# 1005088h/3d_object_detection

Measured on AMD Instinct MI355X. Metric: point-cloud frames/sec end-to-end (voxelise→NMS), eight_20cm, 1x MI355X, higher is better.
Workload: dtype f32; 1 GPU; configs/eight_20cm.json, synthetic KITTI-shape 64-beam 20k-point clouds (mean 20000 points, one distinct cloud per frame of a step), independent frames (batch=1 semantics), random-init weights (InstanceNorm backbone), AABB NMS; `value`: clouds resident in HBM; frames_per_pass_per_gpu=32, engine_max_batch=32, parallelism=frame-sharded x1

## Files before the change

3d_object_detection_amd/csrc/conv.hip:

```cpp
#include <algorithm>
#include <type_traits>
#include <cmath>
#include <cstdio>
#include <cstdlib>
#include <cstring>
#include <unistd.h>
#include "pp_common.h"
#include "conv_common.h"

namespace {

using namespace ppc;

__global__ void __launch_bounds__(256) norm_relu_stats(const float* __restrict__ x, float* __restrict__ y, int C, int HW,
                                                       int pre, const double* __restrict__ pre_acc,
                                                       const float* __restrict__ pre_scale, const float* __restrict__ pre_shift,
                                                       double inv_n, float eps, double* __restrict__ stat_acc,
                                                       size_t x_fs, size_t acc_fs, int x16, int y16)
{
    const int c = blockIdx.y;
    const _Float16* xh = reinterpret_cast<const _Float16*>(x) + blockIdx.z * x_fs;
    _Float16* yh = reinterpret_cast<_Float16*>(y) + blockIdx.z * x_fs;
    x += blockIdx.z * x_fs;
    y += blockIdx.z * x_fs;
// ... 441 lines not shown
        p.feat_fs = (size_t)ctx->cfg.max_voxels * 64;
    }
    const bool fin_in_kernel = B == 1 && finalises_in_prologue(L.var.family);
    if (pre.mode == PRE_STATS && net->aff && L.cin <= 320 && !fin_in_kernel) {
        hipLaunchKernelGGL(norm_finalize, dim3(B), dim3(320), 0, stream, pre.acc, pre.fs, L.cin, pre.inv_n, p.eps, net->aff, (size_t)640);
        p.pre = PRE_AFFINE; p.pre_scale = net->aff; p.pre_shift = net->aff + 320; p.aff_fs = 640;
    }
    const Variant& v = L.var;
    const bool tag = ctx->prof_on && L.kind == 0 && L.level == 0 && L.stride == 1;
    auto prof_begin = [&]() -> int {
        if (!tag) return 0;
        if (ctx->prof_used + 2 > ctx->prof_ev.size()) {
            hipEvent_t a, b;
            PP_HIP(hipEventCreate(&a));
            PP_HIP(hipEventCreate(&b));
            ctx->prof_ev.push_back(a);
            ctx->prof_ev.push_back(b);
        }
        ctx->prof_flops = 2.0 * Hout * Wout * (double)L.cin * L.cout * 9.0 * B;
        PP_HIP(hipEventRecord(ctx->prof_ev[ctx->prof_used], stream));
        return 0;
    };
    auto prof_end = [&]() -> int {
        if (!tag) return 0;
        PP_HIP(hipEventRecord(ctx->prof_ev[ctx->prof_used + 1], stream));
        ctx->prof_used += 2;
        return 0;
    };
    dim3 grid(pp_div_up(Wout, v.pw) * pp_div_up(Hout, v.ph), pp_div_up(L.rows, v.bm), B);
    p.nb = B;
    const size_t lds_bytes = layer_lds(v, L.cin);
    if (v.family == Family::Gemm1x1 && ((Hin * Win) & 3)) return PP_E_ARG;
    if (v.family == Family::Gemm1x1) {
        const int ncb = pp_div_up(L.rows, v.bm);
        int g = (net->num_cu * v.wpc / ncb) * ncb;
        if (g < ncb) g = ncb;
        grid = dim3(g, 1, 1);
    }
    if (v.family == Family::Conv16) {
        if ((size_t)L.rows * Hout * Wout * 4 >= 0x80000000ull || (size_t)L.cin * Hin * Win * 4 >= 0x80000000ull) return PP_E_ARG;
        if (p.pre == PRE_STATS) return pp_fail(ctx, PP_E_STATE, "conv16: the producer's statistics must be finalised to (scale, shift)");
        if ((Win & 3) || (Wout & 3) || (L.cin & 15) || (L.rows % v.bm)) return PP_E_ARG;
        const int total = pp_div_up(Wout, v.pw) * pp_div_up(Hout, v.ph) * (L.rows / v.bm) * B;
        int g = net->num_cu * (v.waves * 64 / v.threads);

        if (g > total) g = total;
        g = (g + 7) & ~7;
        grid = dim3(g, 1, 1);
    }
    if (v.family == Family::Wino4 || v.family == Family::Wino6) {
        if ((size_t)L.rows * Hout * Wout * 4 >= 0x80000000ull) return PP_E_ARG;
        if (p.pre == PRE_RAW) return pp_fail(ctx, PP_E_ARG, "wino4 / wino6 tilings have no raw prologue: give the layer a (scale, shift)");
        const int ncb = pp_div_up(L.rows, v.bm);
        const int2* ts_items = nullptr;
        const int32_t* ts_count = nullptr;
        const bool listed = ts_k > 0 && v.family == Family::Wino6 && v.kern2 && v.pw == 16 && v.ph == 16 && net->eff_prec == 0 && !net->up16 &&
                            L.kind == 0 && L.level == 0 && L.stride == 1 && Wout % v.pw == 0 && Hout % v.ph == 0 && Hout == ctx->H && Wout == ctx->W &&
                            pp_ts_list(ctx, ts_k, B, &ts_items, &ts_count);
        if (tag) {
            const double dense = (double)(Wout / v.pw) * (Hout / v.ph) * ncb * B;
            ctx->prof_items_dense += dense;
            if (listed) ctx->prof_ts_layer.push_back(ts_k | (ncb << 8)); else ctx->prof_items += dense;
        }
        if (int rc = prof_begin()) return rc;
        auto launch_region = [&](const Variant& rv, int x0, int y0, int x1, int y1) {
            ConvP q = p;
// ... 8 lines not shown
        };
        const int mw = (Wout / v.pw) * v.pw, mh = (Hout / v.ph) * v.ph;
        const Variant &sv = strip_v(v.family), &sh = strip_h(v.family);
        const int plan_b = ctx->max_batch;
        auto rounds = [&](int tiles) { return tiles > 0 ? pp_div_up((int64_t)tiles * ncb * plan_b, net->num_cu) : 0; };
        const int t_main = (mw / v.pw) * (mh / v.ph);
        const int t_right = Wout > mw ? pp_div_up(Wout - mw, sv.pw) * pp_div_up(Hout, sv.ph) : 0;
        const int t_bottom = Hout > mh ? pp_div_up(mw, sh.pw) * pp_div_up(Hout - mh, sh.ph) : 0;
        const double tile_us = v.family == Family::Wino6 ? 1.9 * (L.cin / 8) + 3.5 : 2.4 * (L.cin / 8) + 5.0;
        const double full = rounds(pp_div_up(Wout, v.pw) * pp_div_up(Hout, v.ph)) * tile_us;
        const double split = (rounds(t_main) + rounds(t_right) + rounds(t_bottom)) * tile_us + 30.0 * ((t_right > 0) + (t_bottom > 0));
        const bool no_strips = net->w4_strips == 0, all_strips = net->w4_strips == 2;
        if ((split < full || all_strips) && mw > 0 && mh > 0 && !no_strips && (Wout > mw || Hout > mh)) {
            launch_region(v, 0, 0, mw, mh);
            if (Wout > mw) launch_region(sv, mw, 0, Wout, Hout);
            if (Hout > mh) launch_region(sh, 0, mh, mw, Hout);
        } else {
            launch_region(v, 0, 0, Wout, Hout);
            if (listed)
                if (int rc = pp_ts_fill(ctx, ts_k, B, out, p.out_fs, L.rows, stream)) return rc;
        }
        if (int rc = prof_end()) return rc;
        PP_HIP(hipGetLastError());
        return 0;
    }
    if (v.family == Family::Wino) {
        const int total = (int)grid.x * (int)grid.y * B;
        int g = (v.threads >= 512 ? 1 : 2) * net->num_cu;
        if (g > total) g = total;
        g = (g + 7) & ~7;
        grid = dim3(g, 1, 1);
    }
    if (int rc = prof_begin()) return rc;
    hipLaunchKernelGGL((pmap && v.kern2) ? v.kern2 : v.kern, grid, dim3(v.threads), lds_bytes, stream, p);
    if (int rc = prof_end()) return rc;
    PP_HIP(hipGetLastError());
    return 0;
}


__global__ void __launch_bounds__(256) f32_to_f16(const float* __restrict__ x, _Float16* __restrict__ y, size_t n)
{
    for (size_t i = (size_t)blockIdx.x * blockDim.x + threadIdx.x; i < n; i += (size_t)gridDim.x * blockDim.x) y[i] = (_Float16)x[i];
}

__global__ void __launch_bounds__(256) fill_pattern(float* __restrict__ x, size_t n)
{
    for (size_t i = (size_t)blockIdx.x * blockDim.x + threadIdx.x; i < n; i += (size_t)gridDim.x * blockDim.x) {
        unsigned h = (unsigned)i * 2654435761u;
        h ^= h >> 15; h *= 2246822519u; h ^= h >> 13;
        x[i] = (float)(h & 0xFFFF) * (1.0f / 65536.0f);
    }
}

std::map<std::string, std::string>& tune_cache()
{
    static std::map<std::string, std::string> c;
    static bool loaded = false;
    if (!loaded) {
        loaded = true;
        if (const char* path = getenv("PP_TUNE_CACHE")) {
            if (FILE* f = fopen(path, "r")) {
                char line[512];
                while (fgets(line, sizeof(line), f)) {
                    char* tab = strchr(line, '\t');
                    if (!tab) continue;
                    *tab = 0;
// ... 228 lines not shown
    PP_HIP(hipMalloc((void**)&net->bn_scale, (size_t)24 * 320 * sizeof(float)));
    PP_HIP(hipMalloc((void**)&net->bn_shift, (size_t)24 * 320 * sizeof(float)));
    PP_HIP(hipMalloc((void**)&net->head_bias, (size_t)head_rows(ctx->cfg.num_anchor_per_loc) * sizeof(float)));
    PP_HIP(hipMalloc((void**)&net->head_bias_perm, 96 * sizeof(float)));
    PP_HIP(hipMalloc((void**)&net->ones, 320 * sizeof(float)));
    PP_HIP(hipMalloc((void**)&net->zeros, 320 * sizeof(float)));
    std::vector<float> one(320, 1.f);
    PP_HIP(hipMemcpy(net->ones, one.data(), 320 * sizeof(float), hipMemcpyHostToDevice));
    PP_HIP(hipMemset(net->zeros, 0, 320 * sizeof(float)));
    int cin = 64;
    for (int b = 0; b < 3; ++b) {
        const int c = kC[b];
        const int nres[3] = {1, 1, 0};
        const int nunits = (b == 0) ? 2 : 3;
        char key[128];
        snprintf(key, sizeof(key), "rpn.block%d.0.weight", b + 1);
        net->layers.push_back(Layer{key, 0, cin, c, 2, 1, b, pick_variant(0, 2, 1, c, H >> b, W >> b)});
        for (int u = 0; u < nunits; ++u) {
            const int nl = (b == 0) ? (u == 0 ? 1 : 0) : nres[u];
            snprintf(key, sizeof(key), "rpn.block%d.%d.conv_block.2.weight", b + 1, 3 + u);
            net->layers.push_back(Layer{key, 0, c, c, 1, 1, b, pick_variant(0, 1, 1, c, H >> b, W >> b)});
            if (nl == 1) {
                snprintf(key, sizeof(key), "rpn.block%d.%d.conv_block.5.weight", b + 1, 3 + u);
                net->layers.push_back(Layer{key, 0, c, c, 1, 1, b, pick_variant(0, 1, 1, c, H >> b, W >> b)});
            }
        }
        const int up = 1 << b;
        snprintf(key, sizeof(key), "rpn.deconv%d.0.weight", b + 1);
        net->layers.push_back(Layer{key, 1, c, (b == 0) ? 64 : 128, 1, up, b, pick_variant(1, 1, up, ((b == 0) ? 64 : 128) * up * up, H >> b, W >> b)});
        cin = c;
    }
    net->layers.push_back(Layer{"heads", 2, 320, 10 * ctx->cfg.num_anchor_per_loc, 1, 1, 0,
                                pick_variant(2, 1, 1, head_rows(ctx->cfg.num_anchor_per_loc), H, W, ctx->cfg.num_anchor_per_loc == 9)});
    for (Layer& L : net->layers)
        PP_HIP(hipFuncSetAttribute((const void*)L.var.kern, hipFuncAttributeMaxDynamicSharedMemorySize, (int)L.var.lds));
    for (Family f : {Family::Wino4, Family::Wino6})
        for (const Variant* sv : {&strip_v(f), &strip_h(f)})
            PP_HIP(hipFuncSetAttribute((const void*)sv->kern, hipFuncAttributeMaxDynamicSharedMemorySize, (int)sv->lds));
    return 0;
}

void pp_net_destroy(pp_ctx* ctx)
{
    pp_net* net = (pp_net*)ctx->net;
    if (!net) return;
    for (int l = 0; l < 3; ++l)
        for (int b = 0; b < 4; ++b)
            if (net->buf[l][b]) (void)hipFree(net->buf[l][b] - W6_FRONT_PAD);
    for (Layer& L : net->layers)
        if (L.w) (void)hipFree(L.w);
    void* ptrs[] = {net->dbg_stats, net->up, net->stats, net->aff, net->bn_scale, net->bn_shift, net->head_bias, net->head_bias_perm, net->ones, net->zeros};
    for (void* q : ptrs)
        if (q) (void)hipFree(q);
    delete net;
    ctx->net = nullptr;
}

static int fold_bn(pp_ctx* ctx, const std::string& prefix, int C, int site)
{
    pp_net* net = (pp_net*)ctx->net;
    auto get = [&](const char* s) -> const std::vector<float>* {
        auto it = ctx->host_w.find(prefix + s);
        if (it == ctx->host_w.end() || (int)it->second.data.size() != C) return nullptr;
        return &it->second.data;
    };
    const std::vector<float>*g = get(".weight"), *b = get(".bias"), *rm = get(".running_mean"), *rv = get(".running_var");
    if (!g || !b || !rm || !rv) return pp_fail(ctx, PP_E_NAME, ("missing BatchNorm tensors for " + prefix).c_str());
    std::vector<float> sc(C), sh(C);
// ... 30 lines not shown
        float hp[96];
        for (int t = 0; t < 96; ++t) hp[t] = head_tile_row(t) >= 0 ? hb[head_tile_row(t)] : 0.f;
        PP_HIP(hipMemcpy(net->head_bias_perm, hp, sizeof(hp), hipMemcpyHostToDevice));
    }
    {
        const char* at = getenv("PP_AUTOTUNE");
        const char* vb = getenv("PP_VERBOSE");
        const bool tune = !(at && at[0] == '0');
        const bool verbose = vb && vb[0] != '0';
        const int H = ctx->H, W = ctx->W;
        float *tin = nullptr, *tout = nullptr;
        const bool can_tune = tune && (H % 4 == 0) && (W % 4 == 0);
        net->up16 = ctx->precision == 4 && (W % 16 == 0) && ((H * W) % 64 == 0) && ctx->cfg.num_anchor_per_loc == 9;
        net->eff_prec = (ctx->precision == 4 && !net->up16) ? 3 : ctx->precision;
        if (can_tune) {
            const size_t nin = std::max((size_t)64 * ctx->gx * ctx->gy, (size_t)320 * H * W);
            const int tb = ctx->max_batch < TUNE_FRAMES ? ctx->max_batch : TUNE_FRAMES;
            PP_HIP(hipMalloc((void**)&tin, ((size_t)tb * nin + 256 + W6_FRONT_PAD) * sizeof(float)));
            tin += W6_FRONT_PAD;
            PP_HIP(hipMalloc((void**)&tout, ((size_t)tb * 320 * H * W + 256) * sizeof(float)));
            hipLaunchKernelGGL(fill_pattern, dim3(2048), dim3(256), 0, 0, tin, (size_t)tb * nin);
        }
        for (Layer& L : net->layers) {
            int rc = 0;
            {
                const int h = H >> L.level, w = W >> L.level;
                const int hin = (L.kind == 0 && L.stride == 2) ? h * 2 : h, win = (L.kind == 0 && L.stride == 2) ? w * 2 : w;
                if (!can_tune && net->eff_prec == 0) L.var = pick_variant(L.kind, L.stride, L.up, (L.kind == 2) ? head_rows(ctx->cfg.num_anchor_per_loc) : (L.kind == 1 ? L.cout * L.up * L.up : L.cout), h, w, ctx->cfg.num_anchor_per_loc == 9);
                rc = autotune_layer(ctx, L, hin, win, h, w, tin, tout, verbose, can_tune);
                if (rc) { if (tin) { (void)hipFree(tin - W6_FRONT_PAD); (void)hipFree(tout); } return rc; }
            }
            PP_HIP(hipFuncSetAttribute((const void*)L.var.kern, hipFuncAttributeMaxDynamicSharedMemorySize,
                                       (int)layer_lds(L.var, L.cin)));
            if (L.var.kern2) PP_HIP(hipFuncSetAttribute((const void*)L.var.kern2, hipFuncAttributeMaxDynamicSharedMemorySize, (int)L.var.lds));
            rc = pack_layer(ctx, L);
            if (rc) { if (tin) { (void)hipFree(tin - W6_FRONT_PAD); (void)hipFree(tout); } return rc; }
        }
        ctx->sc1_kc = (net->layers[0].var.family == Family::Direct && net->layers[0].var.kc == 8) ? 8 : 4;
        {
            const Layer& head = net->layers.back();
            net->defer_ok = net->eff_prec == 0 && na == 9 && head.var.family == Family::Gemm1x1 && head.var.prec == 0 && head.var.io16 == 0;
            if (net->defer_ok) {
                const int rc = autotune_head_cls(ctx, tin, verbose, can_tune);
                if (rc) { if (tin) { (void)hipFree(tin - W6_FRONT_PAD); (void)hipFree(tout); } return rc; }
            }
        }
        if (tin) { PP_HIP(hipDeviceSynchronize()); (void)hipFree(tin - W6_FRONT_PAD); (void)hipFree(tout); tune_cache_save(); }
        if (net->up16)
            for (const Layer& L : net->layers)
                if ((L.kind == 1 && L.var.io16 != 3) || (L.kind == 2 && L.var.io16 != 1) ||
                    (L.kind == 0 && L.var.io16 != ((L.stride == 2 && L.level == 0) ? 2 : 3)))
                    return pp_fail(ctx, PP_E_STATE, "fp16s: a layer did not get a 16-bit-tensor tiling (PP_FORCE_VARIANT?)");
    }
    if (ctx->cfg.norm_kind == 1) {
        for (int b = 0; b < 3; ++b) {
            char key[128];
            const int c = kC[b];
            snprintf(key, sizeof(key), "rpn.block%d.1", b + 1);
            int rc = fold_bn(ctx, key, c, site_block(b, 0));
            if (rc) return rc;
            const int nunits = (b == 0) ? 2 : 3;
            for (int u = 0; u < nunits; ++u) {
                const int nl = (u == nunits - 1) ? 0 : 1;
                snprintf(key, sizeof(key), "rpn.block%d.%d.conv_block.0", b + 1, 3 + u);
                if ((rc = fold_bn(ctx, key, c, site_block(b, 1 + 2 * u)))) return rc;
                if (nl) {
                    snprintf(key, sizeof(key), "rpn.block%d.%d.conv_block.3", b + 1, 3 + u);
// ... 675 lines not shown
```

3d_object_detection_amd/csrc/gemm1x1.hip:

```cpp
#include <cstdio>
#include "pp_common.h"
#include "conv_common.h"

namespace {

using namespace ppc;

typedef short s16x4 __attribute__((ext_vector_type(4)));
typedef __bf16 bf16x2_t __attribute__((ext_vector_type(2)));
__device__ __forceinline__ unsigned pk_bf16(float a, float b)
{
    return __builtin_bit_cast(unsigned, __builtin_convertvector((f32x2_t){a, b}, bf16x2_t));
}
template <int PREC>
__device__ __forceinline__ f32x4 mfma_lp(const s16x4 a, const s16x4 b, const f32x4 c)
{
    if constexpr (PREC == 3) return __builtin_amdgcn_mfma_f32_16x16x16f16(__builtin_bit_cast(f16x4_t, a), __builtin_bit_cast(f16x4_t, b), c, 0, 0, 0);
    else return __builtin_amdgcn_mfma_f32_16x16x16bf16_1k(a, b, c, 0, 0, 0);
}

template <int MT, int NT, int EPI, int PREC = 0, int IO16 = 0, int PDX = 0>
__global__ void __launch_bounds__(512, EPI == EPI_HEAD_CLS ? 4 : 2) gemm1x1(const ConvP p)
{
    constexpr bool IN16 = (IO16 & 1) != 0, OUT16 = (IO16 & 2) != 0;
    static_assert(IO16 == 0 || PREC != 0, "16-bit storage comes with the 16-bit operand path");
    static_assert(!OUT16 || EPI != EPI_HEAD, "the head's logits stay fp32");
    constexpr int BM = MT * 16;
    constexpr int BMP = BM + ((BM % 32 == 0) ? 16 : 0);
    static_assert(EPI != EPI_HEAD_CLS || (MT == 1 && PREC == 0 && IO16 == 0), "the cls-only head pass is one fp32 M-tile");
    constexpr int PD = PDX ? PDX : (MT >= 8) ? 4 : 8;
    extern __shared__ __attribute__((aligned(16))) float smem[];
    float* wl = smem;
    const int K = p.Cin;
    float* sc_all = wl + (size_t)K * BMP;
    const int tid = threadIdx.x, lane = tid & 63, wave = __builtin_amdgcn_readfirstlane(tid >> 6);
    const int m = lane & 15, kq = lane >> 4;
    float* scl = sc_all + (size_t)wave * 2 * K;
    float* shl = scl + K;

    const int ncb = (p.Cout + BM - 1) / BM;
    const bool xcd_ok = gridDim.x % (8 * ncb) == 0;
    const int xj = blockIdx.x >> 3, xk = blockIdx.x & 7;
    const int cb = xcd_ok ? xj % ncb : blockIdx.x % ncb;
    const int wi = xcd_ok ? xk + 8 * (xj / ncb) : blockIdx.x / ncb, nworkers = gridDim.x / ncb;
    if (wi >= nworkers) return;
    const int co0 = cb * BM;
    if constexpr (EPI == EPI_HEAD_CLS) {
        for (int e = tid; e < K * BMP; e += 512) {
            const int k = e / BMP, a = e - k * BMP, t = 4 * (9 + a) + 3;
            wl[e] = a < p.n_cls ? p.w[((size_t)(t / p.w_bm) * K + k) * p.w_bmp + t % p.w_bm] : 0.f;
        }
    } else {
        const f32x4* g = reinterpret_cast<const f32x4*>(p.w) + (size_t)cb * ((size_t)K * BMP / 4);
        f32x4* d = reinterpret_cast<f32x4*>(wl);
        for (int e = tid; e < K * BMP / 4; e += 512) d[e] = g[e];
    }
// ... 23 lines not shown
                float s = ssum[i][r], q = ssq[i][r];
                s = row16_sum(s);
                q = row16_sum(q);
                const int row = co0 + i * 16 + kq * 4 + r;
                int ch = row;
                bool lead = (m == 0);
                if (EPI == EPI_UP2) { ch = row >> 2; lead = lead && r == 0; }
                if (EPI == EPI_UP4) { ch = row >> 4; lead = lead && r == 0; }
                if (lead && row < p.Cout) {
                    atomicAdd(base + (size_t)ch * 2, (double)s);
                    atomicAdd(base + (size_t)ch * 2 + 1, (double)q);
                }
                ssum[i][r] = 0.f;
                ssq[i][r] = 0.f;
            }
    };

    const int aoff = kq * BMP + m;
    static_assert(NT == 4, "gemm1x1 is written for 4 interleaved N-tiles");
    const int nsteps = K / 4;
    const unsigned bstep = 16u * (unsigned)plane;
    __amdgpu_buffer_rsrc_t rb = __builtin_amdgcn_make_buffer_rsrc(const_cast<float*>(p.in), 0, 0x7FFFFFFF, 0x00020000);
    unsigned bvoff = 0u;
    f32x4 bq[PD];
    auto set_load_item = [&](int it) {
        const int f_ = __builtin_amdgcn_readfirstlane(it / items_per_frame);
        const int px_ = __builtin_amdgcn_readfirstlane((it - f_ * items_per_frame) * (NT * 16)) + 4 * m;
        const uint64_t bp_ = IN16 ? (uint64_t)(reinterpret_cast<const _Float16*>(p.in) + (size_t)f_ * p.in_fs) : (uint64_t)(p.in + (size_t)f_ * p.in_fs);
        const uint64_t bps_ = ((uint64_t)(uint32_t)__builtin_amdgcn_readfirstlane((int)(bp_ >> 32)) << 32) | (uint32_t)__builtin_amdgcn_readfirstlane((int)(uint32_t)bp_);
        rb = __builtin_amdgcn_make_buffer_rsrc(reinterpret_cast<float*>(bps_), 0, 0x7FFFFFFF, 0x00020000);
        bvoff = ((unsigned)kq * (unsigned)plane + (unsigned)(px_ < HW ? px_ : 0)) * (IN16 ? 2u : 4u);
    };
#define G1_LOADB(S, SLOT) bq[SLOT] = __builtin_bit_cast(f32x4, __builtin_amdgcn_raw_buffer_load_b128(rb, bvoff, (unsigned)(S) * bstep, 0));
#define G1_PREP(S, SLOT, PAR)                                                                    \
    {                                                                                            \
        _Pragma("unroll") for (int i = 0; i < MT; ++i) a[PAR][i] = wl[(S) * 4 * BMP + aoff + i * 16]; \
        if (p.pre != PRE_RAW) {                                                                  \
            const float sc = scl[(S) * 4 + kq], sh = shl[(S) * 4 + kq];                          \
            _Pragma("unroll") for (int j = 0; j < NT; ++j) b[PAR][j] = fmaxf(fmaf(bq[SLOT][j], sc, sh), 0.f); \
        } else {                                                                                 \
            _Pragma("unroll") for (int j = 0; j < NT; ++j) b[PAR][j] = bq[SLOT][j];              \
        }                                                                                        \
    }
#define G1_MFMAS(PAR)                                                                            \
    {                                                                                            \
        __builtin_amdgcn_sched_barrier(0);                                                       \
        _Pragma("unroll") for (int i = 0; i < MT; ++i)                                           \
            _Pragma("unroll") for (int j = 0; j < NT; ++j)                                       \
                acc[i][j] = __builtin_amdgcn_mfma_f32_16x16x4f32(a[PAR][i], b[PAR][j], acc[i][j], 0, 0, 0); \
        __builtin_amdgcn_sched_barrier(0);                                                       \
    }
    if constexpr (PREC == 0) {
    if (gw < total) {
        set_load_item(gw);
#pragma unroll
        for (int s0 = 0; s0 < PD - 1; ++s0) G1_LOADB(s0, s0)
    }
    }
    for (int item = gw; item < total; item += gstride) {
        const int fr = __builtin_amdgcn_readfirstlane(item / items_per_frame);
        const int pix0 = __builtin_amdgcn_readfirstlane((item - fr * items_per_frame) * (NT * 16));
        if (fr != stat_frame) { flush_stats(stat_frame); stat_frame = fr; }
        if (p.pre != PRE_RAW && fr != pre_frame) {
            for (int c = lane; c < K; c += 64) {
                if (p.pre == PRE_STATS) {
                    const double* pa = p.pre_acc + (size_t)fr * p.pre_fs;
                    double s = 0.0, q = 0.0;
#pragma unroll
                    for (int r = 0; r < NREP; ++r) { s += pa[((size_t)r * K + c) * 2]; q += pa[((size_t)r * K + c) * 2 + 1]; }
                    const double mean = s * p.pre_inv_n;
                    double var = q * p.pre_inv_n - mean * mean;
                    var = var > 0.0 ? var : 0.0;
                    const double rstd = 1.0 / sqrt(var + (double)p.eps);
                    scl[c] = (float)rstd;
                    shl[c] = (float)(-mean * rstd);
                } else {
                    scl[c] = p.pre_scale[(size_t)fr * p.aff_fs + c];
                    shl[c] = p.pre_shift[(size_t)fr * p.aff_fs + c];
                }
            }
            pre_frame = fr;
        }
        const int pxb = pix0 + 4 * m;
        const bool pok = pxb < HW;
        f32x4 acc[MT][NT];
#pragma unroll
        for (int i = 0; i < MT; ++i)
#pragma unroll
            for (int j = 0; j < NT; ++j) acc[i][j] = (f32x4){0.f, 0.f, 0.f, 0.f};

        if constexpr (PREC == 0) {
        float a[2][MT], b[2][NT];
        G1_PREP(0, 0, 0)
        __builtin_amdgcn_s_setprio(0);
        int sb = 0;
        for (; sb < nsteps - PD; sb += PD) {
#pragma unroll
            for (int u = 0; u < PD; ++u) {
                G1_LOADB(sb + u + PD - 1, (u + PD - 1) % PD)
                G1_PREP(sb + u + 1, (u + 1) % PD, (u + 1) & 1)
                G1_MFMAS(u & 1)
            }
        }
        G1_LOADB(sb + PD - 1, PD - 1)
#pragma unroll
        for (int u = 0; u < PD; ++u) {
            if (u + 1 < PD) G1_PREP(sb + u + 1, (u + 1) % PD, (u + 1) & 1)
            G1_MFMAS(u & 1)
        }

        __builtin_amdgcn_s_setprio(1);
        if (item + gstride < total) {
            set_load_item(item + gstride);
#pragma unroll
            for (int s0 = 0; s0 < PD - 1; ++s0) G1_LOADB(s0, s0)
        }

        } else {
            set_load_item(item);
            constexpr unsigned EB = IN16 ? 2u : 4u;
            const unsigned bvq = bvoff + (unsigned)kq * 3u * (unsigned)plane * EB;
            const unsigned cstep = (unsigned)plane * EB;
            const uint2* wl2 = reinterpret_cast<const uint2*>(wl);
            const int nkb = K / 16;
            f32x4 q0[4], q1[4];
            uint2 g0[4], g1[4];
#define G1_LP_LOAD(Q, G, KB) _Pragma("unroll") for (int t = 0; t < 4; ++t) {                                                  \
        if constexpr (IN16) G[t] = __builtin_bit_cast(uint2, __builtin_amdgcn_raw_buffer_load_b64(rb, bvq, (unsigned)((KB) * 16 + t) * cstep, 0)); \
        else Q[t] = __builtin_bit_cast(f32x4, __builtin_amdgcn_raw_buffer_load_b128(rb, bvq, (unsigned)((KB) * 16 + t) * cstep, 0)); \
    }
#define G1_LP_BLOCK(Q, G, KB, RAW)                                                               \
    {                                                                                            \
        f32x4 sc4 = (f32x4){1.f, 1.f, 1.f, 1.f}, sh4 = (f32x4){0.f, 0.f, 0.f, 0.f};              \
        if constexpr (!(RAW)) { sc4 = *reinterpret_cast<const f32x4*>(scl + (KB) * 16 + kq * 4); sh4 = *reinterpret_cast<const f32x4*>(shl + (KB) * 16 + kq * 4); } \
        s16x4 bh[NT], bl[NT];                                                                    \
        _Pragma("unroll") for (int j = 0; j < NT; ++j) {                                         \
            if constexpr (IN16 && (RAW)) {                                                       \
                const unsigned sel_ = (j & 1) ? 0x07060302u : 0x05040100u;                       \
                const unsigned h0 = __builtin_amdgcn_perm((j & 2) ? G[1].y : G[1].x, (j & 2) ? G[0].y : G[0].x, sel_); \
                const unsigned h1 = __builtin_amdgcn_perm((j & 2) ? G[3].y : G[3].x, (j & 2) ? G[2].y : G[2].x, sel_); \
                bh[j] = __builtin_bit_cast(s16x4, (uint2){h0, h1});                              \
// ... 6 lines not shown
                }                                                                                \
                const unsigned h0 = (PREC == 3) ? pk_f16(v_[0], v_[1]) : pk_bf16(v_[0], v_[1]);  \
                const unsigned h1 = (PREC == 3) ? pk_f16(v_[2], v_[3]) : pk_bf16(v_[2], v_[3]);  \
                bh[j] = __builtin_bit_cast(s16x4, (uint2){h0, h1});                              \
                if constexpr (PREC == 1) {                                                       \
                    const float l0 = v_[0] - __uint_as_float(h0 << 16), l1 = v_[1] - __uint_as_float(h0 & 0xFFFF0000u); \
                    const float l2 = v_[2] - __uint_as_float(h1 << 16), l3 = v_[3] - __uint_as_float(h1 & 0xFFFF0000u); \
                    bl[j] = __builtin_bit_cast(s16x4, (uint2){pk_bf16(l0, l1), pk_bf16(l2, l3)}); \
                }                                                                                \
            }                                                                                    \
        }                                                                                        \
        _Pragma("unroll") for (int i = 0; i < MT; ++i) {                                         \
            const s16x4 ah = __builtin_bit_cast(s16x4, wl2[(((KB) * 2 + 0) * 4 + kq) * BMP + i * 16 + m]); \
            s16x4 al = ah;                                                                       \
            if constexpr (PREC == 1) al = __builtin_bit_cast(s16x4, wl2[(((KB) * 2 + 1) * 4 + kq) * BMP + i * 16 + m]); \
            _Pragma("unroll") for (int j = 0; j < NT; ++j) {                                     \
                acc[i][j] = mfma_lp<PREC>(ah, bh[j], acc[i][j]);                                 \
                if constexpr (PREC == 1) {                                                       \
                    acc[i][j] = mfma_lp<PREC>(ah, bl[j], acc[i][j]);                             \
                    acc[i][j] = mfma_lp<PREC>(al, bh[j], acc[i][j]);                             \
                }                                                                                \
            }                                                                                    \
        }                                                                                        \
    }
#define G1_LP_LOOP(RAW)                                                                          \
    G1_LP_LOAD(q0, g0, 0)                                                                        \
    for (int kb = 0; kb < nkb; kb += 2) {                \
        G1_LP_LOAD(q1, g1, kb + 1)                                                               \
        G1_LP_BLOCK(q0, g0, kb, RAW)                                                             \
        if (kb + 2 < nkb) G1_LP_LOAD(q0, g0, kb + 2)                                             \
        G1_LP_BLOCK(q1, g1, kb + 1, RAW)                                                         \
    }
            __builtin_amdgcn_s_setprio(0);
            if (p.pre == PRE_RAW) { G1_LP_LOOP(true) } else { G1_LP_LOOP(false) }
            __builtin_amdgcn_s_setprio(1);
#undef G1_LP_LOOP
#undef G1_LP_LOAD
#undef G1_LP_BLOCK
        }

        float* gout = OUT16 ? reinterpret_cast<float*>(reinterpret_cast<_Float16*>(p.out) + (size_t)fr * p.out_fs) : p.out + (size_t)fr * p.out_fs;
        auto st4 = [&](size_t off, const f32x4 v) __attribute__((always_inline)) {
            if constexpr (OUT16) {
                const uint2 h = {pk_f16(v[0], v[1]), pk_f16(v[2], v[3])};
                *reinterpret_cast<uint2*>(reinterpret_cast<_Float16*>(gout) + off) = h;
            } else {
                *reinterpret_cast<f32x4*>(gout + off) = v;
            }
        };
        float* gbox = p.out_box ? p.out_box + (size_t)fr * p.box_fs : nullptr;
        float* gdir = p.out_dir ? p.out_dir + (size_t)fr * p.dir_fs : nullptr;
        bool up4_done = false;
        if constexpr (EPI == EPI_UP4) {
            if ((p.Wout & 3) == 0) {
                up4_done = true;
                int kq_e = kq;
                asm volatile("" : "+v"(kq_e));
                const int t_ = m & 3;
                size_t ko[4];
                bool kok[4];
#pragma unroll
                for (int k = 0; k < 4; ++k) {
                    const int pk = pix0 + 4 * ((m & ~3) + k);
                    const int yk = pk / p.Wout, xk = pk - yk * p.Wout;
                    kok[k] = pk < HW;
                    ko[k] = (size_t)(4 * yk) * ((size_t)p.Wout * 4) + 4 * (size_t)xk + 4 * t_;
                }
#pragma unroll
                for (int i = 0; i < MT; ++i) {
                    const int row0 = co0 + i * 16 + kq_e * 4;
                    if (row0 >= p.Cout) continue;
                    const int co = row0 >> 4, dy = (row0 >> 2) & 3;
                    f32x4 o4[4];
#pragma unroll
                    for (int r = 0; r < 4; ++r) {
                        float a0 = acc[i][0][r], a1 = acc[i][1][r], a2 = acc[i][2][r], a3 = acc[i][3][r];
                        if (pok) {
                            ssum[i][0] += (a0 + a1) + (a2 + a3);
                            ssq[i][0] += (a0 * a0 + a1 * a1) + (a2 * a2 + a3 * a3);
                        }
                        const float x0 = dpp_f32<0xB1>(a1), x1 = dpp_f32<0xB1>(a0), x2 = dpp_f32<0xB1>(a3), x3 = dpp_f32<0xB1>(a2);
                        const bool odd = t_ & 1, hi = t_ & 2;
                        const float c0 = odd ? x0 : a0, c1 = odd ? a1 : x1, c2 = odd ? x2 : a2, c3 = odd ? a3 : x3;
                        const float z0 = dpp_f32<0x4E>(c2), z1 = dpp_f32<0x4E>(c3), z2 = dpp_f32<0x4E>(c0), z3 = dpp_f32<0x4E>(c1);
                        o4[0][r] = hi ? z0 : c0; o4[1][r] = hi ? z1 : c1; o4[2][r] = hi ? c2 : z2; o4[3][r] = hi ? c3 : z3;
                    }
                    const size_t ob = (size_t)co * plane * 16 + (size_t)dy * ((size_t)p.Wout * 4);
#pragma unroll
                    for (int k = 0; k < 4; ++k)
                        if (kok[k]) st4(ob + ko[k], o4[k]);
                }
            }
        }
        if (pok && !up4_done) {
            int kq_e = kq;
            asm volatile("" : "+v"(kq_e));
            const bool row4 = (p.Wout & 3) == 0;
            const int py_ = pxb / p.Wout, px_ = pxb - py_ * p.Wout;
            (void)row4; (void)py_; (void)px_;
#pragma unroll
            for (int i = 0; i < MT; ++i) {
                const int row0 = co0 + i * 16 + kq_e * 4;
                if (row0 >= p.Cout) continue;
                if (EPI == EPI_PLAIN) {
#pragma unroll
                    for (int r = 0; r < 4; ++r) {
                        const f32x4 x = (f32x4){acc[i][0][r], acc[i][1][r], acc[i][2][r], acc[i][3][r]};
                        st4((size_t)(row0 + r) * plane + pxb, x);
                        ssum[i][r] += (x[0] + x[1]) + (x[2] + x[3]);
                        ssq[i][r] += (x[0] * x[0] + x[1] * x[1]) + (x[2] * x[2] + x[3] * x[3]);
                    }
                } else if (EPI == EPI_UP2) {
                    const int co = row0 >> 2;
                    const size_t W2 = (size_t)p.Wout * 2;
                    if (row4) {
                        const size_t o = (size_t)co * plane * 4 + (size_t)(2 * py_) * W2 + 2 * px_;
                        st4(o, (f32x4){acc[i][0][0], acc[i][0][1], acc[i][1][0], acc[i][1][1]});
                        st4(o + 4, (f32x4){acc[i][2][0], acc[i][2][1], acc[i][3][0], acc[i][3][1]});
                        st4(o + W2, (f32x4){acc[i][0][2], acc[i][0][3], acc[i][1][2], acc[i][1][3]});
                        st4(o + W2 + 4, (f32x4){acc[i][2][2], acc[i][2][3], acc[i][3][2], acc[i][3][3]});
#pragma unroll
                        for (int j = 0; j < NT; ++j)
#pragma unroll
                            for (int r = 0; r < 4; ++r) { ssum[i][0] += acc[i][j][r]; ssq[i][0] += acc[i][j][r] * acc[i][j][r]; }
                    } else {
#pragma unroll
                        for (int j = 0; j < NT; ++j) {
                            const int y = (pxb + j) / p.Wout, xx = (pxb + j) - y * p.Wout;
                            const f32x4 v = acc[i][j];
                            float* o = gout + (size_t)co * plane * 4 + (size_t)(2 * y) * W2 + 2 * xx;
                            *reinterpret_cast<float2*>(o) = make_float2(v[0], v[1]);
                            *reinterpret_cast<float2*>(o + W2) = make_float2(v[2], v[3]);
#pragma unroll
                            for (int r = 0; r < 4; ++r) { ssum[i][0] += v[r]; ssq[i][0] += v[r] * v[r]; }
                        }
                    }
                } else if (EPI == EPI_UP4) {
                    const int co = row0 >> 4, dy = (row0 >> 2) & 3;
                    const size_t W4o = (size_t)p.Wout * 4;
#pragma unroll
                    for (int j = 0; j < NT; ++j) {
                        const int y = row4 ? py_ : (pxb + j) / p.Wout, xx = row4 ? px_ + j : (pxb + j) - y * p.Wout;
                        const f32x4 v = acc[i][j];
                        float* o = gout + (size_t)co * plane * 16 + (size_t)(4 * y + dy) * W4o + 4 * xx;
                        *reinterpret_cast<float4*>(o) = make_float4(v[0], v[1], v[2], v[3]);
#pragma unroll
                        for (int r = 0; r < 4; ++r) { ssum[i][0] += v[r]; ssq[i][0] += v[r] * v[r]; }
                    }
// ... 20 lines not shown
                        const int a_ = g - 9;
#pragma unroll
                        for (int j = 0; j < NT; ++j) {
                            float* o = gbox + ((size_t)a_ * plane + pxb + j) * 7 + 4;
                            *reinterpret_cast<f32x2u*>(o) = (f32x2u){acc[i][j][0] + bs[0], acc[i][j][1] + bs[1]};
                            o[2] = acc[i][j][2] + bs[2];
                        }
                        *reinterpret_cast<f32x4*>(gout + (size_t)a_ * plane + pxb) =
                            (f32x4){acc[i][0][3] + bs[3], acc[i][1][3] + bs[3], acc[i][2][3] + bs[3], acc[i][3][3] + bs[3]};
                    } else if (g < 23) {
                        const int a0 = 2 * (g - 18);
#pragma unroll
                        for (int j = 0; j < NT; ++j) {
                            *reinterpret_cast<float2*>(gdir + ((size_t)a0 * plane + pxb + j) * 2) = make_float2(acc[i][j][0] + bs[0], acc[i][j][1] + bs[1]);
                            if (a0 + 1 < 9)
                                *reinterpret_cast<float2*>(gdir + ((size_t)(a0 + 1) * plane + pxb + j) * 2) = make_float2(acc[i][j][2] + bs[2], acc[i][j][3] + bs[3]);
                        }
                    }
                }
            }
        }
    }
    flush_stats(stat_frame);
#undef G1_MFMAS
#undef G1_PREP
#undef G1_LOADB
}

template <int MT, int NT, int EPI, int PREC = 0, int IO16 = 0>
Variant make_g1()
{
    Variant v;
    v.kern = gemm1x1<MT, NT, EPI, PREC, IO16>;
    v.prec = PREC;
    v.io16 = IO16;
    v.bm = MT * 16; v.bmp = v.bm + ((v.bm % 32 == 0) ? 16 : 0); v.pw = NT * 16; v.ph = 1; v.kc = 4; v.threads = 512;
    v.waves = 8; v.pairs = MT * NT;
    v.lds = 0;
    v.family = Family::Gemm1x1;
    if (IO16) snprintf(v.name, sizeof(v.name), "g1x1 m%d n%d e%d h%d p%d", MT, NT, EPI, IO16, PREC);
    else if (PREC) snprintf(v.name, sizeof(v.name), "g1x1 m%d n%d e%d p%d", MT, NT, EPI, PREC);
    else snprintf(v.name, sizeof(v.name), "g1x1 m%d n%d e%d", MT, NT, EPI);
    return v;
}

template <int PD>
Variant make_g1_cls()
{
    Variant v;
    v.kern = gemm1x1<1, 4, EPI_HEAD_CLS, 0, 0, PD>;
    v.bm = 16; v.bmp = 16; v.pw = 64; v.ph = 1; v.kc = 4; v.threads = 512;
    v.waves = 8; v.pairs = 4;
    v.lds = 0;
    v.family = Family::Gemm1x1;
    v.wpc = 2;
    snprintf(v.name, sizeof(v.name), "g1x1 cls pd%d wg%d", PD, v.wpc);
    return v;
}

template <int PREC, bool S16 = false>
void lp_menu(int kind, int up, std::vector<Variant>& menu)
{
    constexpr int HI = S16 ? 1 : 0, DO = S16 ? 3 : 0;
    if (kind == 2) { menu.push_back(make_g1<6, 4, EPI_HEAD, PREC, HI>()); menu.push_back(make_g1<3, 4, EPI_HEAD, PREC, HI>()); }
    else if (up == 1) { menu.push_back(make_g1<4, 4, EPI_PLAIN, PREC, DO>()); menu.push_back(make_g1<2, 4, EPI_PLAIN, PREC, DO>()); }
    else if (up == 2) { menu.push_back(make_g1<4, 4, EPI_UP2, PREC, DO>()); menu.push_back(make_g1<8, 4, EPI_UP2, PREC, DO>()); }
// ... 27 lines not shown
```

Before: 1098 frames/s.

## Add raw-input gemm1x1 twin and lean buffer-store epilogues for fp32 path

Builds a second fp32 gemm1x1 instantiation that skips the per-k scale/shift/ReLU prologue and feeds loaded B operands straight into the MFMAs. Dispatch picks this twin when the input is raw. The fp32 main loop now walks incremental weight and scale pointers, and the plain/up2/up4 epilogues use 32-bit-offset buffer stores, a DPP quad transpose in inline asm, and paired-float statistics math to cut address arithmetic and branches. The cost is an extra kernel per variant and a 2GB output-size limit on the lean path, with out-of-bounds handling via the buffer descriptor's range.

After: 1103 frames/s, median of 6. About the same (+0.5%).

```diff
diff --git a/3d_object_detection_amd/csrc/conv.hip b/3d_object_detection_amd/csrc/conv.hip
--- a/3d_object_detection_amd/csrc/conv.hip
+++ b/3d_object_detection_amd/csrc/conv.hip
@@ -497,6 +497,7 @@
     const size_t lds_bytes = layer_lds(v, L.cin);
     if (v.family == Family::Gemm1x1 && ((Hin * Win) & 3)) return PP_E_ARG;
     if (v.family == Family::Gemm1x1) {
+        if (L.kind == 1 && v.prec == 0 && (size_t)L.rows * Hout * Wout * 4 >= 0x80000000ull) return PP_E_ARG;
         const int ncb = pp_div_up(L.rows, v.bm);
         int g = (net->num_cu * v.wpc / ncb) * ncb;
         if (g < ncb) g = ncb;
@@ -571,7 +572,9 @@
         grid = dim3(g, 1, 1);
     }
     if (int rc = prof_begin()) return rc;
-    hipLaunchKernelGGL((pmap && v.kern2) ? v.kern2 : v.kern, grid, dim3(v.threads), lds_bytes, stream, p);
+    if (v.family == Family::Gemm1x1 && v.prec == 0 && p.pre == PRE_RAW && !v.kern2) return pp_fail(ctx, PP_E_ARG, "this gemm1x1 tiling has no raw twin: give the layer a (scale, shift)");
+    const bool twin = v.kern2 && (v.family == Family::Gemm1x1 ? p.pre == PRE_RAW : pmap != nullptr);
+    hipLaunchKernelGGL(twin ? v.kern2 : v.kern, grid, dim3(v.threads), lds_bytes, stream, p);
     if (int rc = prof_end()) return rc;
     PP_HIP(hipGetLastError());
     return 0;
@@ -866,8 +869,10 @@
     }
     net->layers.push_back(Layer{"heads", 2, 320, 10 * ctx->cfg.num_anchor_per_loc, 1, 1, 0,
                                 pick_variant(2, 1, 1, head_rows(ctx->cfg.num_anchor_per_loc), H, W, ctx->cfg.num_anchor_per_loc == 9)});
-    for (Layer& L : net->layers)
+    for (Layer& L : net->layers) {
         PP_HIP(hipFuncSetAttribute((const void*)L.var.kern, hipFuncAttributeMaxDynamicSharedMemorySize, (int)L.var.lds));
+        if (L.var.kern2) PP_HIP(hipFuncSetAttribute((const void*)L.var.kern2, hipFuncAttributeMaxDynamicSharedMemorySize, (int)L.var.lds));
+    }
     for (Family f : {Family::Wino4, Family::Wino6})
         for (const Variant* sv : {&strip_v(f), &strip_h(f)})
             PP_HIP(hipFuncSetAttribute((const void*)sv->kern, hipFuncAttributeMaxDynamicSharedMemorySize, (int)sv->lds));
@@ -964,7 +969,7 @@
             }
             PP_HIP(hipFuncSetAttribute((const void*)L.var.kern, hipFuncAttributeMaxDynamicSharedMemorySize,
                                        (int)layer_lds(L.var, L.cin)));
-            if (L.var.kern2) PP_HIP(hipFuncSetAttribute((const void*)L.var.kern2, hipFuncAttributeMaxDynamicSharedMemorySize, (int)L.var.lds));
+            if (L.var.kern2) PP_HIP(hipFuncSetAttribute((const void*)L.var.kern2, hipFuncAttributeMaxDynamicSharedMemorySize, (int)layer_lds(L.var, L.cin)));
             rc = pack_layer(ctx, L);
             if (rc) { if (tin) { (void)hipFree(tin - W6_FRONT_PAD); (void)hipFree(tout); } return rc; }
         }
diff --git a/3d_object_detection_amd/csrc/gemm1x1.hip b/3d_object_detection_amd/csrc/gemm1x1.hip
--- a/3d_object_detection_amd/csrc/gemm1x1.hip
+++ b/3d_object_detection_amd/csrc/gemm1x1.hip
@@ -7,6 +7,34 @@
 using namespace ppc;
 
 typedef short s16x4 __attribute__((ext_vector_type(4)));
+typedef unsigned u32x4_t __attribute__((ext_vector_type(4)));
+__device__ __forceinline__ void quad_transpose4(float a0, float a1, float a2, float a3, float& o0, float& o1, float& o2, float& o3)
+{
+    float c0, c1, c2, c3;
+    asm("s_nop 1\n\t"
+        "s_mov_b32 vcc_lo, 0xaaaaaaaa\n\t"
+        "s_mov_b32 vcc_hi, 0xaaaaaaaa\n\t"
+        "v_cndmask_b32_dpp %1, %8, %9, vcc quad_perm:[1,0,3,2] row_mask:0xf bank_mask:0xf\n\t"
+        "v_cndmask_b32_dpp %3, %10, %11, vcc quad_perm:[1,0,3,2] row_mask:0xf bank_mask:0xf\n\t"
+        "s_not_b64 vcc, vcc\n\t"
+        "v_cndmask_b32_dpp %0, %9, %8, vcc quad_perm:[1,0,3,2] row_mask:0xf bank_mask:0xf\n\t"
+        "v_cndmask_b32_dpp %2, %11, %10, vcc quad_perm:[1,0,3,2] row_mask:0xf bank_mask:0xf\n\t"
+        "s_mov_b32 vcc_lo, 0xcccccccc\n\t"
+        "s_mov_b32 vcc_hi, 0xcccccccc\n\t"
+        "v_cndmask_b32_dpp %7, %1, %3, vcc quad_perm:[2,3,0,1] row_mask:0xf bank_mask:0xf\n\t"
+        "v_cndmask_b32_dpp %6, %0, %2, vcc quad_perm:[2,3,0,1] row_mask:0xf bank_mask:0xf\n\t"
+        "s_not_b64 vcc, vcc\n\t"
+        "v_cndmask_b32_dpp %4, %2, %0, vcc quad_perm:[2,3,0,1] row_mask:0xf bank_mask:0xf\n\t"
+        "v_cndmask_b32_dpp %5, %3, %1, vcc quad_perm:[2,3,0,1] row_mask:0xf bank_mask:0xf"
+        : "=&v"(c0), "=&v"(c1), "=&v"(c2), "=&v"(c3), "=&v"(o0), "=&v"(o1), "=&v"(o2), "=&v"(o3)
+        : "v"(a0), "v"(a1), "v"(a2), "v"(a3)
+        : "vcc", "scc");
+}
+template <int CTRL>
+__device__ __forceinline__ unsigned dpp_u32(unsigned v)
+{
+    return (unsigned)__builtin_amdgcn_update_dpp(0, (int)v, CTRL, 0xF, 0xF, true);
+}
 typedef __bf16 bf16x2_t __attribute__((ext_vector_type(2)));
 __device__ __forceinline__ unsigned pk_bf16(float a, float b)
 {
@@ -19,9 +47,11 @@
     else return __builtin_amdgcn_mfma_f32_16x16x16bf16_1k(a, b, c, 0, 0, 0);
 }
 
-template <int MT, int NT, int EPI, int PREC = 0, int IO16 = 0, int PDX = 0>
+template <int MT, int NT, int EPI, int PREC = 0, int IO16 = 0, int PDX = 0, bool RAWT = false>
 __global__ void __launch_bounds__(512, EPI == EPI_HEAD_CLS ? 4 : 2) gemm1x1(const ConvP p)
 {
+    static_assert(!RAWT || PREC == 0, "the raw twin is the fp32 loop's");
+    const bool raw = PREC == 0 ? RAWT : p.pre == PRE_RAW;
     constexpr bool IN16 = (IO16 & 1) != 0, OUT16 = (IO16 & 2) != 0;
     static_assert(IO16 == 0 || PREC != 0, "16-bit storage comes with the 16-bit operand path");
     static_assert(!OUT16 || EPI != EPI_HEAD, "the head's logits stay fp32");
@@ -111,22 +141,20 @@
         bvoff = ((unsigned)kq * (unsigned)plane + (unsigned)(px_ < HW ? px_ : 0)) * (IN16 ? 2u : 4u);
     };
 #define G1_LOADB(S, SLOT) bq[SLOT] = __builtin_bit_cast(f32x4, __builtin_amdgcn_raw_buffer_load_b128(rb, bvoff, (unsigned)(S) * bstep, 0));
-#define G1_PREP(S, SLOT, PAR)                                                                    \
+#define G1_PREP(U, SLOT, PAR)                                                                    \
     {                                                                                            \
-        _Pragma("unroll") for (int i = 0; i < MT; ++i) a[PAR][i] = wl[(S) * 4 * BMP + aoff + i * 16]; \
-        if (p.pre != PRE_RAW) {                                                                  \
-            const float sc = scl[(S) * 4 + kq], sh = shl[(S) * 4 + kq];                          \
+        _Pragma("unroll") for (int i = 0; i < MT; ++i) a[PAR][i] = wa[(U) * 4 * BMP + i * 16];   \
+        if constexpr (!RAWT) {                                                                   \
+            const float sc = sca[(U) * 4], sh = sca[K + (U) * 4];                                \
             _Pragma("unroll") for (int j = 0; j < NT; ++j) b[PAR][j] = fmaxf(fmaf(bq[SLOT][j], sc, sh), 0.f); \
-        } else {                                                                                 \
-            _Pragma("unroll") for (int j = 0; j < NT; ++j) b[PAR][j] = bq[SLOT][j];              \
         }                                                                                        \
     }
-#define G1_MFMAS(PAR)                                                                            \
+#define G1_MFMAS(SLOT, PAR)                                                                      \
     {                                                                                            \
         __builtin_amdgcn_sched_barrier(0);                                                       \
         _Pragma("unroll") for (int i = 0; i < MT; ++i)                                           \
             _Pragma("unroll") for (int j = 0; j < NT; ++j)                                       \
-                acc[i][j] = __builtin_amdgcn_mfma_f32_16x16x4f32(a[PAR][i], b[PAR][j], acc[i][j], 0, 0, 0); \
+                acc[i][j] = __builtin_amdgcn_mfma_f32_16x16x4f32(a[PAR][i], RAWT ? bq[SLOT][j] : b[PAR][j], acc[i][j], 0, 0, 0); \
         __builtin_amdgcn_sched_barrier(0);                                                       \
     }
     if constexpr (PREC == 0) {
@@ -140,7 +168,7 @@
         const int fr = __builtin_amdgcn_readfirstlane(item / items_per_frame);
         const int pix0 = __builtin_amdgcn_readfirstlane((item - fr * items_per_frame) * (NT * 16));
         if (fr != stat_frame) { flush_stats(stat_frame); stat_frame = fr; }
-        if (p.pre != PRE_RAW && fr != pre_frame) {
+        if (!raw && fr != pre_frame) {
             for (int c = lane; c < K; c += 64) {
                 if (p.pre == PRE_STATS) {
                     const double* pa = p.pre_acc + (size_t)fr * p.pre_fs;
@@ -170,6 +198,9 @@
 
         if constexpr (PREC == 0) {
         float a[2][MT], b[2][NT];
+        const float* wa = wl + aoff;
+        const float* sca = scl + kq;
+        (void)b; (void)sca;
         G1_PREP(0, 0, 0)
         __builtin_amdgcn_s_setprio(0);
         int sb = 0;
@@ -177,15 +208,17 @@
 #pragma unroll
             for (int u = 0; u < PD; ++u) {
                 G1_LOADB(sb + u + PD - 1, (u + PD - 1) % PD)
-                G1_PREP(sb + u + 1, (u + 1) % PD, (u + 1) & 1)
-                G1_MFMAS(u & 1)
+                G1_PREP(u + 1, (u + 1) % PD, (u + 1) & 1)
+                G1_MFMAS(u, u & 1)
             }
+            wa += PD * 4 * BMP;
+            sca += PD * 4;
         }
         G1_LOADB(sb + PD - 1, PD - 1)
 #pragma unroll
         for (int u = 0; u < PD; ++u) {
-            if (u + 1 < PD) G1_PREP(sb + u + 1, (u + 1) % PD, (u + 1) & 1)
-            G1_MFMAS(u & 1)
+            if (u + 1 < PD) G1_PREP(u + 1, (u + 1) % PD, (u + 1) & 1)
+            G1_MFMAS(u, u & 1)
         }
 
         __builtin_amdgcn_s_setprio(1);
@@ -258,7 +291,7 @@
         G1_LP_BLOCK(q1, g1, kb + 1, RAW)                                                         \
     }
             __builtin_amdgcn_s_setprio(0);
-            if (p.pre == PRE_RAW) { G1_LP_LOOP(true) } else { G1_LP_LOOP(false) }
+            if (raw) { G1_LP_LOOP(true) } else { G1_LP_LOOP(false) }
             __builtin_amdgcn_s_setprio(1);
 #undef G1_LP_LOOP
 #undef G1_LP_LOAD
@@ -276,6 +309,13 @@
         };
         float* gbox = p.out_box ? p.out_box + (size_t)fr * p.box_fs : nullptr;
         float* gdir = p.out_dir ? p.out_dir + (size_t)fr * p.dir_fs : nullptr;
+        constexpr bool LEAN = PREC == 0 && (EPI == EPI_PLAIN || EPI == EPI_UP2 || EPI == EPI_UP4);
+        constexpr unsigned G1_FAR = 0x80000000u;
+        __amdgpu_buffer_rsrc_t ro = __builtin_amdgcn_make_buffer_rsrc(gout, 0, 0x7FFFFFFF, 0x00020000);
+        auto stb = [&](unsigned voff, unsigned soff, const f32x4 v) __attribute__((always_inline)) {
+            __builtin_amdgcn_raw_buffer_store_b128(__builtin_bit_cast(u32x4_t, v), ro, voff + soff, 0, 0);
+        };
+        (void)G1_FAR; (void)stb;
         bool up4_done = false;
         if constexpr (EPI == EPI_UP4) {
             if ((p.Wout & 3) == 0) {
@@ -283,38 +323,73 @@
                 int kq_e = kq;
                 asm volatile("" : "+v"(kq_e));
                 const int t_ = m & 3;
-                size_t ko[4];
-                bool kok[4];
-#pragma unroll
-                for (int k = 0; k < 4; ++k) {
-                    const int pk = pix0 + 4 * ((m & ~3) + k);
-                    const int yk = pk / p.Wout, xk = pk - yk * p.Wout;
-                    kok[k] = pk < HW;
-                    ko[k] = (size_t)(4 * yk) * ((size_t)p.Wout * 4) + 4 * (size_t)xk + 4 * t_;
-                }
-#pragma unroll
-                for (int i = 0; i < MT; ++i) {
-                    const int row0 = co0 + i * 16 + kq_e * 4;
-                    if (row0 >= p.Cout) continue;
-                    const int co = row0 >> 4, dy = (row0 >> 2) & 3;
-                    f32x4 o4[4];
-#pragma unroll
-                    for (int r = 0; r < 4; ++r) {
-                        float a0 = acc[i][0][r], a1 = acc[i][1][r], a2 = acc[i][2][r], a3 = acc[i][3][r];
+                if constexpr (LEAN) {
+                    const int y_ = pxb / p.Wout, x_ = pxb - y_ * p.Wout;
+                    const unsigned W16 = (unsigned)p.Wout * 16u;
+                    const unsigned own = pok ? (unsigned)(4 * y_) * W16 + (unsigned)x_ * 16u : G1_FAR;
+                    const unsigned mine = (unsigned)kq_e * W16 + 16u * (unsigned)t_;
+                    const unsigned ko[4] = {dpp_u32<0x00>(own) + mine, dpp_u32<0x55>(own) + mine, dpp_u32<0xAA>(own) + mine, dpp_u32<0xFF>(own) + mine};
+                    const unsigned cstride = (unsigned)plane * 64u;
+#pragma unroll
+                    for (int i = 0; i < MT; ++i) {
+                        const int row0 = co0 + i * 16 + kq_e * 4;
+                        if (row0 >= p.Cout) continue;
                         if (pok) {
-                            ssum[i][0] += (a0 + a1) + (a2 + a3);
-                            ssq[i][0] += (a0 * a0 + a1 * a1) + (a2 * a2 + a3 * a3);
-                        }
-                        const float x0 = dpp_f32<0xB1>(a1), x1 = dpp_f32<0xB1>(a0), x2 = dpp_f32<0xB1>(a3), x3 = dpp_f32<0xB1>(a2);
-                        const bool odd = t_ & 1, hi = t_ & 2;
-                        const float c0 = odd ? x0 : a0, c1 = odd ? a1 : x1, c2 = odd ? x2 : a2, c3 = odd ? a3 : x3;
-                        const float z0 = dpp_f32<0x4E>(c2), z1 = dpp_f32<0x4E>(c3), z2 = dpp_f32<0x4E>(c0), z3 = dpp_f32<0x4E>(c1);
-                        o4[0][r] = hi ? z0 : c0; o4[1][r] = hi ? z1 : c1; o4[2][r] = hi ? c2 : z2; o4[3][r] = hi ? c3 : z3;
-                    }
-                    const size_t ob = (size_t)co * plane * 16 + (size_t)dy * ((size_t)p.Wout * 4);
-#pragma unroll
-                    for (int k = 0; k < 4; ++k)
-                        if (kok[k]) st4(ob + ko[k], o4[k]);
+#pragma unroll
+                            for (int r = 0; r < 4; r += 2) {
+                                const f32x2_t a0 = {acc[i][0][r], acc[i][0][r + 1]}, a1 = {acc[i][1][r], acc[i][1][r + 1]};
+                                const f32x2_t a2 = {acc[i][2][r], acc[i][2][r + 1]}, a3 = {acc[i][3][r], acc[i][3][r + 1]};
+                                const f32x2_t s2 = (a0 + a1) + (a2 + a3);
+                                const f32x2_t q2 = (a0 * a0 + a1 * a1) + (a2 * a2 + a3 * a3);
+                                ssum[i][0] += s2[0]; ssq[i][0] += q2[0];
+                                ssum[i][0] += s2[1]; ssq[i][0] += q2[1];
+                            }
+                        }
+                        f32x4 o4[4];
+#pragma unroll
+                        for (int r = 0; r < 4; ++r) {
+                            float t0, t1, t2, t3;
+                            quad_transpose4(acc[i][0][r], acc[i][1][r], acc[i][2][r], acc[i][3][r], t0, t1, t2, t3);
+                            o4[0][r] = t0; o4[1][r] = t1; o4[2][r] = t2; o4[3][r] = t3;
+                        }
+                        const unsigned so = (unsigned)(co0 / 16 + i) * cstride;
+#pragma unroll
+                        for (int k = 0; k < 4; ++k) stb(ko[k], so, o4[k]);
+                    }
+                } else {
+                    size_t ko[4];
+                    bool kok[4];
+#pragma unroll
+                    for (int k = 0; k < 4; ++k) {
+                        const int pk = pix0 + 4 * ((m & ~3) + k);
+                        const int yk = pk / p.Wout, xk = pk - yk * p.Wout;
+                        kok[k] = pk < HW;
+                        ko[k] = (size_t)(4 * yk) * ((size_t)p.Wout * 4) + 4 * (size_t)xk + 4 * t_;
+                    }
+#pragma unroll
+                    for (int i = 0; i < MT; ++i) {
+                        const int row0 = co0 + i * 16 + kq_e * 4;
+                        if (row0 >= p.Cout) continue;
+                        const int co = row0 >> 4, dy = (row0 >> 2) & 3;
+                        f32x4 o4[4];
+#pragma unroll
+                        for (int r = 0; r < 4; ++r) {
+                            float a0 = acc[i][0][r], a1 = acc[i][1][r], a2 = acc[i][2][r], a3 = acc[i][3][r];
+                            if (pok) {
+                                ssum[i][0] += (a0 + a1) + (a2 + a3);
+                                ssq[i][0] += (a0 * a0 + a1 * a1) + (a2 * a2 + a3 * a3);
+                            }
+                            const float x0 = dpp_f32<0xB1>(a1), x1 = dpp_f32<0xB1>(a0), x2 = dpp_f32<0xB1>(a3), x3 = dpp_f32<0xB1>(a2);
+                            const bool odd = t_ & 1, hi = t_ & 2;
+                            const float c0 = odd ? x0 : a0, c1 = odd ? a1 : x1, c2 = odd ? x2 : a2, c3 = odd ? a3 : x3;
+                            const float z0 = dpp_f32<0x4E>(c2), z1 = dpp_f32<0x4E>(c3), z2 = dpp_f32<0x4E>(c0), z3 = dpp_f32<0x4E>(c1);
+                            o4[0][r] = hi ? z0 : c0; o4[1][r] = hi ? z1 : c1; o4[2][r] = hi ? c2 : z2; o4[3][r] = hi ? c3 : z3;
+                        }
+                        const size_t ob = (size_t)co * plane * 16 + (size_t)dy * ((size_t)p.Wout * 4);
+#pragma unroll
+                        for (int k = 0; k < 4; ++k)
+                            if (kok[k]) st4(ob + ko[k], o4[k]);
+                    }
                 }
             }
         }
@@ -328,7 +403,20 @@
             for (int i = 0; i < MT; ++i) {
                 const int row0 = co0 + i * 16 + kq_e * 4;
                 if (row0 >= p.Cout) continue;
-                if (EPI == EPI_PLAIN) {
+                if constexpr (LEAN && EPI == EPI_PLAIN) {
+                    const unsigned vo = ((unsigned)(kq_e * 4) * (unsigned)plane + (unsigned)pxb) * 4u;
+#pragma unroll
+                    for (int r = 0; r < 4; r += 2) {
+                        const f32x2_t a0 = {acc[i][0][r], acc[i][0][r + 1]}, a1 = {acc[i][1][r], acc[i][1][r + 1]};
+                        const f32x2_t a2 = {acc[i][2][r], acc[i][2][r + 1]}, a3 = {acc[i][3][r], acc[i][3][r + 1]};
+                        stb(vo, (unsigned)(co0 + i * 16 + r) * ((unsigned)plane * 4u), (f32x4){a0[0], a1[0], a2[0], a3[0]});
+                        stb(vo, (unsigned)(co0 + i * 16 + r + 1) * ((unsigned)plane * 4u), (f32x4){a0[1], a1[1], a2[1], a3[1]});
+                        const f32x2_t s2 = (a0 + a1) + (a2 + a3);
+                        const f32x2_t q2 = (a0 * a0 + a1 * a1) + (a2 * a2 + a3 * a3);
+                        ssum[i][r] += s2[0]; ssum[i][r + 1] += s2[1];
+                        ssq[i][r] += q2[0]; ssq[i][r + 1] += q2[1];
+                    }
+                } else if (EPI == EPI_PLAIN) {
 #pragma unroll
                     for (int r = 0; r < 4; ++r) {
                         const f32x4 x = (f32x4){acc[i][0][r], acc[i][1][r], acc[i][2][r], acc[i][3][r]};
@@ -339,7 +427,25 @@
                 } else if (EPI == EPI_UP2) {
                     const int co = row0 >> 2;
                     const size_t W2 = (size_t)p.Wout * 2;
-                    if (row4) {
+                    if (LEAN && row4) {
+                        const unsigned W8 = (unsigned)p.Wout * 8u;
+                        const unsigned vo = (unsigned)kq_e * ((unsigned)plane * 16u) + (unsigned)(2 * py_) * W8 + (unsigned)px_ * 8u;
+                        const unsigned so = (unsigned)(co0 / 4 + i * 4) * ((unsigned)plane * 16u);
+                        stb(vo, so, (f32x4){acc[i][0][0], acc[i][0][1], acc[i][1][0], acc[i][1][1]});
+                        stb(vo + 16u, so, (f32x4){acc[i][2][0], acc[i][2][1], acc[i][3][0], acc[i][3][1]});
+                        stb(vo + W8, so, (f32x4){acc[i][0][2], acc[i][0][3], acc[i][1][2], acc[i][1][3]});
+                        stb(vo + W8 + 16u, so, (f32x4){acc[i][2][2], acc[i][2][3], acc[i][3][2], acc[i][3][3]});
+#pragma unroll
+                        for (int j = 0; j < NT; ++j) {
+                            const f32x2_t lo = {acc[i][j][0], acc[i][j][1]}, hi = {acc[i][j][2], acc[i][j][3]};
+                            f32x2_t ql = lo * lo, qh = hi * hi;
+                            asm("" : "+v"(ql), "+v"(qh));
+                            ssum[i][0] += lo[0]; ssq[i][0] += ql[0];
+                            ssum[i][0] += lo[1]; ssq[i][0] += ql[1];
+                            ssum[i][0] += hi[0]; ssq[i][0] += qh[0];
+                            ssum[i][0] += hi[1]; ssq[i][0] += qh[1];
+                        }
+                    } else if (row4) {
                         const size_t o = (size_t)co * plane * 4 + (size_t)(2 * py_) * W2 + 2 * px_;
                         st4(o, (f32x4){acc[i][0][0], acc[i][0][1], acc[i][1][0], acc[i][1][1]});
                         st4(o + 4, (f32x4){acc[i][2][0], acc[i][2][1], acc[i][3][0], acc[i][3][1]});
@@ -426,6 +532,7 @@
 {
     Variant v;
     v.kern = gemm1x1<MT, NT, EPI, PREC, IO16>;
+    if constexpr (PREC == 0) v.kern2 = gemm1x1<MT, NT, EPI, PREC, IO16, 0, true>;
     v.prec = PREC;
     v.io16 = IO16;
     v.bm = MT * 16; v.bmp = v.bm + ((v.bm % 32 == 0) ? 16 : 0); v.pw = NT * 16; v.ph = 1; v.kc = 4; v.threads = 512;
```
